# hyperledger-labs/bdls

Hardware: AMD Instinct MI355X
Metric: P-256 ECDSA verifies/sec (fused SHA-256, bit-exact vs Go crypto/ecdsa + Fabric low-S) (higher is better)
Workload: dtype u32; 1 GPU; BASELINE config 2: 1048576 records/GPU, 256B messages, 65536 distinct keys, 1/16 corrupted, fused SHA-256; records_per_gpu=1048576, records_total=1048576, msg_len=256, nkeys=65536, corrupt_den=16, parallelism=shard1 (no collective)

## Files before the change

bdls_amd/csrc/ec30.h:

```cpp
#pragma once
#include "fp30.h"

namespace bh {

struct J30 {
  uint32_t X[9], Y[9], Z[9];
};

BH_HD void j_copy(J30& r, const J30& p) {
  f_copy(r.X, p.X);
  f_copy(r.Y, p.Y);
  f_copy(r.Z, p.Z);
}

BH_HD void j_sel(J30& r, bool c, const J30& a, const J30& b) {
  f_sel(r.X, c, a.X, b.X);
  f_sel(r.Y, c, a.Y, b.Y);
  f_sel(r.Z, c, a.Z, b.Z);
}

template <class F>
BH_HD void j_dbl(J30& r, const J30& p) {
  if constexpr (F::a_is_minus3) {
    uint32_t delta[9], gamma[9], bt[9], t0[9], t1[9], u[9], alpha[9];
// ... 109 lines not shown
  f_mul<F>(t3, t2, t3);
  f_sub<F, 32>(r.Y, t3, p.Y);
  f_mul<F>(r.Z, p.Z, t1);
  f_copy(p.X, w1);
  f_copy(p.Z, r.Z);
}

template <class F>
BH_HD bool j_degenerate(const uint32_t z3[9], const uint32_t rr[9], bool* same_y) {
  const bool degenerate = f_is_zero2<F>(z3);
  if (degenerate) {
    uint32_t t[9];
    f_reduce<F>(t, rr);
    uint32_t z = 0;
    for (int i = 0; i < 9; i++) z |= t[i];
    *same_y = (z == 0);
  } else {
    *same_y = false;
  }
  return degenerate;
}

template <class F, bool FUSE = true>
BH_HD void j_zaddc(J30& r, const uint32_t x1[9], const uint32_t y1[9], const uint32_t x2[9],
                   const uint32_t dx[9], const uint32_t sy[9], const uint32_t z[9]) {
  uint32_t c[9], w1[9], w2[9], t2[9], d[9], t3[9], t4[9];
  f_sqr<F>(c, dx);
  f_mul<F>(w1, x1, c);
  f_mul<F>(w2, x2, c);
  f_dblsub<F, 32>(t2, y1, sy);
  f_sqr<F>(d, t2);
  f_sub2<F, 32>(r.X, d, w1, w2);
  f_sub<F, 64>(t3, w1, r.X);
  if constexpr (F::sparse_p256 && FUSE) {
    f_sub<F, 32>(t4, w2, w1);
    f_mul2<F>(r.Y, t2, t3, y1, t4);
  } else {
    f_sub<F, 32>(t4, w1, w2);
    f_mul<F>(t4, y1, t4);
    f_mul<F>(t3, t2, t3);
    f_sub<F, 32>(r.Y, t3, t4);
  }
  f_mul<F>(r.Z, z, dx);
}

template <class F, bool DA>
BH_HD bool j_add_impl(J30& r, const J30& p, const J30& q, bool neg, bool* same_y) {
  uint32_t z1z1[9], z2z2[9], u1[9], u2[9], s1[9], s2[9], h[9], rr[9], t[9], hh[9], hhh[9], w[9];
  f_sqr<F>(z1z1, p.Z);
  f_sqr<F>(z2z2, q.Z);
  f_mul<F>(u1, p.X, z2z2);
  f_mul<F>(u2, q.X, z1z1);
  f_mul<F>(t, q.Z, z2z2);
  f_mul<F>(s1, p.Y, t);
  f_mul<F>(t, p.Z, z1z1);
  f_mul<F>(s2, q.Y, t);
  f_sub<F, 32>(h, u2, u1);
  f_csub<F, 32>(rr, neg, s2, s1);
  f_sqr<F>(hh, h);
  f_mul<F>(hhh, hh, h);
  f_mul<F>(u1, u1, hh);
  f_sqr<F>(t, rr);
  f_add2x(w, hhh, u1);
  if constexpr (DA) {
    uint32_t x3[9], z3[9];
    f_sub<F, 32>(x3, t, w);
    f_addsub<F, 32>(u2, w, u1, t);
    f_mul<F>(s2, rr, u2);
    f_mul<F>(s1, s1, hhh);
    f_mul<F>(t, p.Z, q.Z);
    f_mul<F>(z3, t, h);
    if (j_degenerate<F>(z3, rr, same_y)) return true;
    j_zaddc<F, false>(r, u1, s1, x3, u2, s2, z3);
    return false;
  } else {
    f_sub<F, 32>(r.X, t, w);
    f_addsub<F, 32>(u2, w, u1, t);
    if constexpr (F::sparse_p256) {
      f_neg<F, 32>(s2, s1);
      f_mul2<F>(r.Y, rr, u2, s2, hhh);
    } else {
      f_mul<F>(u2, rr, u2);
      f_mul<F>(s1, s1, hhh);
      f_sub<F, 32>(r.Y, u2, s1);
    }
    f_mul<F>(t, p.Z, q.Z);
    f_mul<F>(r.Z, t, h);
    return j_degenerate<F>(r.Z, rr, same_y);
  }
}

template <class F>
BH_HD bool j_add(J30& r, const J30& p, const J30& q, bool* same_y) {
  return j_add_impl<F, false>(r, p, q, false, same_y);
}
template <class F>
BH_HD bool j_add_da(J30& r, const J30& p, const J30& q, bool* same_y, bool neg = false) {
  return j_add_impl<F, true>(r, p, q, neg, same_y);
}

template <class F, bool DA>
BH_HD bool j_madd_impl(J30& r, const J30& p, const uint32_t x2[9], const uint32_t y2[9], bool neg,
                       bool* same_y) {
  uint32_t z1z1[9], u2[9], s2[9], h[9], rr[9], t[9], hh[9], hhh[9], v[9], w[9];
  f_sqr<F>(z1z1, p.Z);
  f_mul<F>(u2, x2, z1z1);
  f_mul<F>(t, p.Z, z1z1);
  f_mul<F>(s2, y2, t);
  f_sub<F, 64>(h, u2, p.X);
  f_csub<F, 96>(rr, neg, s2, p.Y);
  f_sqr<F>(hh, h);
  f_mul<F>(hhh, hh, h);
  f_mul<F>(v, p.X, hh);
  f_sqr<F>(t, rr);
  f_add2x(w, hhh, v);
  if constexpr (DA) {
    uint32_t x3[9], z3[9];
    f_sub<F, 32>(x3, t, w);
    f_addsub<F, 32>(u2, w, v, t);
    f_mul<F>(s2, rr, u2);
    f_mul<F>(t, p.Y, hhh);
    f_mul<F>(z3, p.Z, h);
    if (j_degenerate<F>(z3, rr, same_y)) return true;
    j_zaddc<F>(r, v, t, x3, u2, s2, z3);
    return false;
  } else {
    f_sub<F, 32>(r.X, t, w);
    f_addsub<F, 32>(s2, w, v, t);
    if constexpr (F::sparse_p256) {
      f_negk<F, 96>(u2, p.Y);
      f_mul2<F>(r.Y, rr, s2, u2, hhh);
    } else {
      f_mul<F>(s2, rr, s2);
      f_mul<F>(t, p.Y, hhh);
      f_sub<F, 32>(r.Y, s2, t);
    }
    f_mul<F>(r.Z, p.Z, h);
    return j_degenerate<F>(r.Z, rr, same_y);
  }
}

template <class F>
BH_HD bool j_madd(J30& r, const J30& p, const uint32_t x2[9], const uint32_t y2[9], bool* same_y,
                  bool neg = false) {
  return j_madd_impl<F, false>(r, p, x2, y2, neg, same_y);
}
template <class F>
BH_HD bool j_madd_da(J30& r, const J30& p, const uint32_t x2[9], const uint32_t y2[9],
                     bool* same_y, bool neg = false) {
  return j_madd_impl<F, true>(r, p, x2, y2, neg, same_y);
}

template <class F>
BH_HD bool j_on_curve(const uint32_t x[9], const uint32_t y[9]) {
  uint32_t l[9], rhs[9], t[9], b[9];
  f_sqr<F>(l, y);
  f_sqr<F>(t, x);
  f_mul<F>(rhs, t, x);
  if constexpr (F::a_is_minus3) {
    f_mulc<3>(t, x);
    f_sub<F, 32>(rhs, rhs, t);
  }
  f_const(b, F::b_m);
  f_add(rhs, rhs, b);
  f_reduce<F>(rhs, rhs);
  f_canon<F>(l, l);
  return f_eq(l, rhs);
}

}
```

bdls_amd/csrc/verify.h:

```cpp
#pragma once
#include <type_traits>

#include "blake2b.h"
#include "der.h"
#include "fe.h"
#include "ec30.h"
#include "sha256.h"
#include "sha3.h"

namespace bh {

enum : uint32_t {
  BHF_HASH_SHA256 = 1u,
  BHF_NO_LOW_S = 2u,
  BHF_HASH_SHA3_256 = 8u,
  BHF_BDLS_PREHASHED = 0x100u,
};

enum : int { HK_GIVEN_OR_SHA256 = 0, HK_SHA3_256 = 1 };

enum : uint8_t { ST_R2OK = 0x80u };

struct BatchIn {
  const uint8_t* pub;
// ... 85 lines not shown
#endif
constexpr int kGW = BH_GCOMB_BITS;
static_assert(kGW >= 8 && kGW <= 14, "G comb window width");
constexpr int kCombWindows = (257 + kGW - 1) / kGW;
constexpr int kCombEntries = 1 << (kGW - 1);
static_assert(kCombWindows * kGW <= 288, "recoded scalar fits 9 limbs");
constexpr int kGEntry = 18;
constexpr int kQTab = 16;
constexpr int kQPt = 28;

struct alignas(16) W4 {
  uint32_t x, y, z, w;
};

#ifndef BH_AOS
#define BH_AOS 1
#endif
BH_HD void ld8(uint32_t v[8], const uint32_t* base, uint32_t i, uint32_t ns) {
#if BH_AOS
  const W4* p = reinterpret_cast<const W4*>(base + (size_t)i * 8);
  const W4 a = p[0], b = p[1];
  v[0] = a.x; v[1] = a.y; v[2] = a.z; v[3] = a.w;
  v[4] = b.x; v[5] = b.y; v[6] = b.z; v[7] = b.w;
#else
#pragma unroll
  for (int k = 0; k < 8; k++) v[k] = base[(size_t)k * ns + i];
#endif
}
BH_HD void st8(uint32_t* base, uint32_t i, uint32_t ns, const uint32_t v[8]) {
#if BH_AOS
  W4* p = reinterpret_cast<W4*>(base + (size_t)i * 8);
  p[0] = W4{v[0], v[1], v[2], v[3]};
  p[1] = W4{v[4], v[5], v[6], v[7]};
#else
#pragma unroll
  for (int k = 0; k < 8; k++) base[(size_t)k * ns + i] = v[k];
#endif
}
BH_HD void ld9(uint32_t v[9], const uint32_t* base, uint32_t i, uint32_t ns) {
#pragma unroll
  for (int k = 0; k < 9; k++) v[k] = BH_AOS ? base[(size_t)i * 9 + k] : base[(size_t)k * ns + i];
}
BH_HD void st9(uint32_t* base, uint32_t i, uint32_t ns, const uint32_t v[9]) {
#pragma unroll
  for (int k = 0; k < 9; k++) (BH_AOS ? base[(size_t)i * 9 + k] : base[(size_t)k * ns + i]) = v[k];
}

template <class P, class C>
BH_HD bool key_import(const uint8_t* q, uint32_t qx30[9], uint32_t qy30[9]) {
  uint32_t qx[8], qy[8], pp[8];
  load_const8(pp, C::p);
  be32_to_limbs(qx, q);
  be32_to_limbs(qy, q + 32);
  if (geq8(qx, pp) || geq8(qy, pp)) return false;
  f_from_u256(qx30, qx);
  f_from_u256(qy30, qy);
  f_to_mont<P>(qx30, qx30);
  f_to_mont<P>(qy30, qy30);
  f_canon<P>(qx30, qx30);
  f_canon<P>(qy30, qy30);
  return j_on_curve<P>(qx30, qy30);
}

template <class P, class C>
BH_HD void stage_prep_key(const BatchIn& in, const Work& w, uint32_t i) {
  uint32_t qx30[9], qy30[9];
  const bool ok = key_import<P, C>(in.pub + (size_t)i * 64, qx30, qy30);
  if (!ok) {
    f_const(qx30, P::gx_m);
    f_const(qy30, P::gy_m);
  }
  st9(w.qx, i, w.ns, qx30);
  st9(w.qy, i, w.ns, qy30);
  w.st[i] = ok ? (uint8_t)R_OK : (uint8_t)R_BAD_KEY;
}

template <class C, int HK>
BH_HD void digest_e(const BatchIn& in, uint32_t i, uint32_t e[8]) {
  const uint32_t mlen = in.msg_len[i];
  const bool fused = HK == HK_SHA3_256 || (in.flags & BHF_HASH_SHA256) != 0;
  const uint8_t* m = in.msg + in.msg_off[i];
  const uint32_t mlen2 = in.msg2_len ? in.msg2_len[i] : 0u;
  if constexpr (HK == HK_SHA3_256) {
    uint8_t hb[32];
    if (mlen2) sha3_256_msg2(hb, m, mlen, in.msg + in.msg2_off[i], mlen2);
    else sha3_256_msg(hb, m, mlen);
    be32_to_limbs(e, hb);
  } else if (fused) {
    uint32_t h[8];
    if (mlen2) sha256_msg2(h, m, mlen, in.msg + in.msg2_off[i], mlen2);
    else sha256_msg(h, m, mlen);
#pragma unroll
    for (int k = 0; k < 8; k++) e[k] = h[7 - k];
  } else {
    const uint32_t L = mlen < 32 ? mlen : 32;
#pragma unroll
    for (int k = 0; k < 8; k++) e[k] = 0;
#pragma unroll
    for (int j = 0; j < 32; j++) {
      uint32_t v = 0;
      if ((uint32_t)j < L) v = m[L - 1 - j];
      e[j >> 2] |= v << (8 * (j & 3));
    }
  }
  uint32_t nn[8], t[8];
  load_const8(nn, C::n);
  const uint32_t bo = sub8(t, e, nn);
  if (!bo) copy8(e, t);
}

template <class P, class N, class C, int HK = HK_GIVEN_OR_SHA256, bool DEFER = false>
BH_HD void stage_prep(const BatchIn& in, const Work& w, uint32_t i) {
  uint8_t reason = R_OK;
  uint32_t r[8], s[8], e[8];
  uint32_t qx30[9], qy30[9];
  const uint32_t slen = in.sig_len[i];
  const uint32_t mlen = in.msg_len[i];
  const bool fused = HK == HK_SHA3_256 || (in.flags & BHF_HASH_SHA256) != 0;
  if (slen == 0) reason = R_EMPTY_SIG;
  else if (!fused && mlen == 0) reason = R_EMPTY_DIGEST;
  DerSig ds;
  if (reason == R_OK) reason = der_parse_sig(in.sig + in.sig_off[i], slen, &ds);
  uint32_t half[8], nn[8];
  load_const8(half, C::half_n);
  load_const8(nn, C::n);
  if (reason == R_OK) {
    copy8(r, ds.r);
    copy8(s, ds.s);
    if (!(in.flags & BHF_NO_LOW_S) && (ds.s_big || !geq8(half, s))) reason = R_HIGH_S;
  }
  if (reason == R_OK && !key_import<P, C>(in.pub + (size_t)i * 64, qx30, qy30))
    reason = R_BAD_KEY;
  if (reason == R_OK && (ds.r_big || geq8(r, nn))) reason = R_R_RANGE;
  if (reason == R_OK && (ds.s_big || geq8(s, nn))) reason = R_S_RANGE;
  if (reason == R_OK && !DEFER) digest_e<C, HK>(in, i, e);
  uint8_t st = reason;
  if (reason == R_OK) {
    uint32_t pmn[8], rn[8], rm[9], r2m[9];
    load_const8(pmn, C::p_minus_n);
    f_from_u256(rm, r);
    f_to_mont<P>(rm, rm);
    f_canon<P>(rm, rm);
    if (!geq8(r, pmn)) {
      st |= ST_R2OK;
      add8(rn, r, nn);
      f_from_u256(r2m, rn);
      f_to_mont<P>(r2m, r2m);
      f_canon<P>(r2m, r2m);
    } else {
      f_copy(r2m, rm);
    }
    st9(w.rm, i, w.ns, rm);
    st9(w.r2m, i, w.ns, r2m);
    to_mont<N>(s, s);
  } else {
    for (int k = 0; k < 8; k++) { e[k] = r[k] = 0; }
    e[0] = r[0] = 1;
    load_const8(s, N::r1);
    f_const(qx30, P::gx_m);
    f_const(qy30, P::gy_m);
  }
  if (!DEFER) st8(w.e, i, w.ns, e);
  st8(w.r, i, w.ns, r);
  st8(w.sm, i, w.ns, s);
  st9(w.qx, i, w.ns, qx30);
  st9(w.qy, i, w.ns, qy30);
  w.st[i] = st;
}

BH_HD void setbytes_u256(const uint8_t* b, uint32_t len, uint32_t v[8], bool* big, bool* zero) {
  uint32_t lo = 0;
  while (lo < len && b[lo] == 0) lo++;
  const uint32_t L = len - lo;
  *zero = (L == 0);
  *big = (L > 32);
#pragma unroll
  for (int k = 0; k < 8; k++) v[k] = 0;
  if (L > 32) return;
#pragma unroll
  for (int j = 0; j < 32; j++) {
    uint32_t x = 0;
    if ((uint32_t)j < L) x = b[len - 1 - j];
    v[j >> 2] |= x << (8 * (j & 3));
  }
}

template <class C>
BH_HD void stage_bdls_given(const BdlsIn& in, const Work& w, uint32_t i) {
  uint32_t e[8], nn[8], t[8];
  const uint8_t* m = in.msg + in.msg_off[i];
  const uint32_t mlen = in.msg_len[i];
  const uint32_t L = mlen < 32 ? mlen : 32;
#pragma unroll
  for (int k = 0; k < 8; k++) e[k] = 0;
#pragma unroll
  for (int j = 0; j < 32; j++) {
    uint32_t v = 0;
    if ((uint32_t)j < L) v = m[L - 1 - j];
    e[j >> 2] |= v << (8 * (j & 3));
  }
  load_const8(nn, C::n);
  if (!sub8(t, e, nn)) copy8(e, t);
  st8(w.e, i, w.ns, e);
}

template <class C>
BH_HD void stage_bdls_hash(const BdlsIn& in, const Work& w, uint32_t i) {
  if (in.flags & BHF_BDLS_PREHASHED) return stage_bdls_given<C>(in, w, i);
  uint8_t hsh[32];
  uint32_t e[8], nn[8], t[8];
  const uint8_t* q = in.xy + (size_t)i * 64;
  bdls_signed_proto_hash(hsh, in.version[i], q, q + 32, in.msg + in.msg_off[i], in.msg_len[i]);
  be32_to_limbs(e, hsh);
  load_const8(nn, C::n);
  if (!sub8(t, e, nn)) copy8(e, t);
  st8(w.e, i, w.ns, e);
}

template <class P, class N, class C>
BH_HD void stage_prep(const BdlsIn& in, const Work& w, uint32_t i) {
  uint8_t reason = R_OK;
  uint32_t r[8], s[8], nn[8];
  uint32_t qx30[9], qy30[9];
  load_const8(nn, C::n);
  bool rbig, rzero, sbig, szero;
  setbytes_u256(in.r + in.r_off[i], in.r_len[i], r, &rbig, &rzero);
  setbytes_u256(in.s + in.s_off[i], in.s_len[i], s, &sbig, &szero);
  if (rzero) reason = R_R_NONPOS;
  else if (szero) reason = R_S_NONPOS;
  const uint8_t* q = in.xy + (size_t)i * 64;
  const bool badkey = reason == R_OK && !key_import<P, C>(q, qx30, qy30);
  if (badkey && P::a_is_minus3) reason = R_BAD_KEY;
  if (reason == R_OK && (rbig || geq8(r, nn))) reason = R_R_RANGE;
  if (reason == R_OK && (sbig || geq8(s, nn))) reason = R_S_RANGE;
  if (reason == R_OK && badkey) reason = R_MATH;
  uint8_t st = reason;
  if (reason == R_OK) {
    uint32_t pmn[8], rn[8], rm[9], r2m[9];
    load_const8(pmn, C::p_minus_n);
    f_from_u256(rm, r);
    f_to_mont<P>(rm, rm);
    f_canon<P>(rm, rm);
    if (!geq8(r, pmn)) {
      st |= ST_R2OK;
      add8(rn, r, nn);
      f_from_u256(r2m, rn);
      f_to_mont<P>(r2m, r2m);
      f_canon<P>(r2m, r2m);
    } else {
      f_copy(r2m, rm);
    }
    st9(w.rm, i, w.ns, rm);
    st9(w.r2m, i, w.ns, r2m);
    to_mont<N>(s, s);
  } else {
    for (int k = 0; k < 8; k++) r[k] = 0;
    r[0] = 1;
    load_const8(s, N::r1);
    f_const(qx30, P::gx_m);
    f_const(qy30, P::gy_m);
  }
  st8(w.r, i, w.ns, r);
  st8(w.sm, i, w.ns, s);
  st9(w.qx, i, w.ns, qx30);
  st9(w.qy, i, w.ns, qy30);
  w.st[i] = st;
}

template <class N, bool U1 = true, bool VAR = false>
BH_HD void stage_inv(const Work& w, uint32_t c, uint32_t stride, uint32_t n) {
  uint32_t acc[8], x[8];
  load_const8(acc, N::r1);
  uint32_t last = c;
  for (uint32_t i = c; i < n; i += stride) {
    st8(w.pre, i, w.ns, acc);
    ld8(x, w.sm, i, w.ns);
    mont_mul<N>(acc, acc, x);
    last = i;
  }
  if (c >= n) return;
  uint32_t inv[8];
  mont_inv_sg<N, VAR>(inv, acc);
  for (uint32_t i = last;; i -= stride) {
    uint32_t pre[8], wi[8], t[8];
    ld8(pre, w.pre, i, w.ns);
    mont_mul<N>(wi, inv, pre);
    ld8(x, w.sm, i, w.ns);
    mont_mul<N>(inv, inv, x);
    if constexpr (U1) {
      ld8(t, w.e, i, w.ns);
      mont_mul<N>(t, t, wi);
      st8(w.e, i, w.ns, t);
    } else {
      st8(w.sm, i, w.ns, wi);
    }
    ld8(t, w.r, i, w.ns);
    mont_mul<N>(t, t, wi);
    st8(w.r, i, w.ns, t);
    if (i < c + stride) break;
  }
}

template <class N>
BH_HD void calc_u1(uint32_t u1[8], const Work& w, uint32_t i) {
  uint32_t wi[8];
  ld8(u1, w.e, i, w.ns);
  ld8(wi, w.sm, i, w.ns);
  mont_mul<N>(u1, u1, wi);
}

BH_HD void booth5(uint32_t in6, uint32_t* mag, bool* neg) {
  uint32_t sgn = 0u - (in6 >> 5);
  uint32_t d = (63u - in6) & sgn;
  d |= in6 & ~sgn;
  *mag = (d >> 1) + (d & 1u);
  *neg = sgn != 0;
}


BH_HD uint32_t* qtab_entry(uint32_t* tab, uint32_t wave, uint32_t entry, uint32_t lane) {
  return tab + (((size_t)wave * 64 + lane) * kQTab + entry) * kQPt;
}

BH_HD void qtab_store(uint32_t* tab, uint32_t wave, uint32_t entry, uint32_t lane, const J30& P) {
  uint32_t v[28];
#pragma unroll
  for (int k = 0; k < 9; k++) {
    v[k] = P.X[k];
    v[9 + k] = P.Y[k];
    v[18 + k] = P.Z[k];
  }
  v[27] = 0;
  W4* d = reinterpret_cast<W4*>(qtab_entry(tab, wave, entry, lane));
#pragma unroll
  for (int q = 0; q < 7; q++) d[q] = W4{v[4 * q], v[4 * q + 1], v[4 * q + 2], v[4 * q + 3]};
}

BH_HD void qtab_load(J30& P, const uint32_t* tab, uint32_t wave, uint32_t entry, uint32_t lane) {
  const W4* s = reinterpret_cast<const W4*>(qtab_entry(const_cast<uint32_t*>(tab), wave, entry, lane));
  uint32_t v[28];
#pragma unroll
  for (int q = 0; q < 7; q++) {
    const W4 t = s[q];
    v[4 * q] = t.x;
    v[4 * q + 1] = t.y;
    v[4 * q + 2] = t.z;
    v[4 * q + 3] = t.w;
  }
#pragma unroll
  for (int k = 0; k < 9; k++) {
    P.X[k] = v[k];
    P.Y[k] = v[9 + k];
    P.Z[k] = v[18 + k];
  }
}

template <class P>
BH_HD void gtab_entry(uint32_t t, uint32_t* out) {
  const uint32_t win = t / kCombEntries, j = t % kCombEntries;
  J30 B;
  f_const(B.X, P::gx_m);
  f_const(B.Y, P::gy_m);
  f_const(B.Z, P::r1);
  for (uint32_t d = 0; d < (uint32_t)kGW * win; d++) j_dbl<P>(B, B);
  const uint32_t k = j + 1;
  int top = 31;
  while (!((k >> top) & 1u)) top--;
  J30 A;
  j_copy(A, B);
  for (int b = top - 1; b >= 0; b--) {
    j_dbl<P>(A, A);
    if ((k >> b) & 1u) {
      bool same;
      J30 R;
      j_add<P>(R, A, B, &same);
      j_copy(A, R);
    }
  }
  uint32_t zi[9], zi2[9], x[9], y[9], z[9];
  f_reduce<P>(z, A.Z);
  f_inv<P>(zi, z);
  f_sqr<P>(zi2, zi);
  f_mul<P>(x, A.X, zi2);
  f_mul<P>(zi2, zi2, zi);
  f_mul<P>(y, A.Y, zi2);
  f_reduce<P>(x, x);
  f_reduce<P>(y, y);
  for (int q = 0; q < 9; q++) {
    out[q] = x[q];
    out[9 + q] = y[q];
  }
}

template <int B>
BH_HD void shr_const(uint32_t v[9]) {
  constexpr int ws = B / 32, bs = B % 32;
#pragma unroll
  for (int q = 0; q < 9; q++) {
    const uint32_t lo = (q + ws < 9) ? v[q + ws] : 0u;
    const uint32_t hi = (q + ws + 1 < 9) ? v[q + ws + 1] : 0u;
    if constexpr (bs != 0) v[q] = (lo >> bs) | (hi << (32 - bs));
    else v[q] = lo;
  }
}

struct GOff {
  uint32_t v[9];
};
constexpr GOff make_goff() {
  GOff o{};
  for (int w = 0; w < kCombWindows; w++) {
    const int b = w * kGW + kGW - 1;
    o.v[b / 32] |= 1u << (b % 32);
  }
  return o;
}
constexpr GOff kGOff = make_goff();

BH_HD void recode_goff(uint32_t v[9], const uint32_t k[8]) {
  uint64_t c = 0;
#pragma unroll
  for (int q = 0; q < 8; q++) {
    c += (uint64_t)k[q] + kGOff.v[q];
    v[q] = (uint32_t)c;
    c >>= 32;
  }
  v[8] = (uint32_t)c + kGOff.v[8];
}

#ifndef BH_GCOMB_PREFETCH
#define BH_GCOMB_PREFETCH 1
#endif
BH_HD void g_window(uint32_t v[9], int win, const uint32_t* gtab, uint32_t tx[9], uint32_t ty[9],
                    uint32_t& mag, bool& neg) {
  const int d = (int)(v[0] & (2u * kCombEntries - 1u)) - kCombEntries;
// ... 875 lines not shown
constexpr size_t kG2Words = (size_t)(kG2Ent + kG1Ent + kGBase) * kLLAff;
constexpr size_t kGCombWords = (size_t)kCombWindows * kCombEntries * kGEntry;
constexpr size_t kGTabAllWords = kGCombWords + kG2Words;
static_assert(kGCombWords % 4 == 0, "folded tables 16-byte aligned");
BH_HD const uint32_t* g2_of(const uint32_t* gtab) { return gtab + kGCombWords; }

template <class P>
BH_HD void scalar_g_affine(const uint32_t v[9], uint32_t x[9], uint32_t y[9]) {
  uint32_t gx[9], gy[9];
  f_const(gx, P::gx_m);
  f_const(gy, P::gy_m);
  int topbit = 287;
  while (topbit > 0 && !((v[topbit >> 5] >> (topbit & 31)) & 1u)) topbit--;
  J30 A;
  f_copy(A.X, gx);
  f_copy(A.Y, gy);
  f_const(A.Z, P::r1);
  for (int b = topbit - 1; b >= 0; b--) {
    j_dbl<P>(A, A);
    if ((v[b >> 5] >> (b & 31)) & 1u) {
      bool same;
      (void)j_madd<P>(A, A, gx, gy, &same);
    }
  }
  uint32_t z[9], zi[9], zi2[9];
  f_reduce<P>(z, A.Z);
  f_inv<P>(zi, z);
  f_sqr<P>(zi2, zi);
  f_mul<P>(x, A.X, zi2);
  f_mul<P>(zi2, zi2, zi);
  f_mul<P>(y, A.Y, zi2);
  f_reduce<P>(x, x);
  f_reduce<P>(y, y);
}

template <class P>
BH_HD void gtab2_base(uint32_t k, uint32_t* g2) {
  const uint32_t i = k / kGOdd, m = k % kGOdd;
  uint32_t v[9] = {0, 0, 0, 0, 0, 0, 0, 0, 0};
  const int b = kLLSpace * (int)i;
  const uint64_t mag = (uint64_t)(2u * m + 1u) << (b & 31);
  v[b >> 5] = (uint32_t)mag;
  if ((b >> 5) + 1 < 9) v[(b >> 5) + 1] = (uint32_t)(mag >> 32);
  uint32_t x[9], y[9];
  scalar_g_affine<P>(v, x, y);
  llaff_store(g2, kG2Ent + kG1Ent + k, x, y);
}

template <class P>
BH_HD void gtab2_entry(uint32_t t, uint32_t* g2) {
  constexpr uint32_t top = 1u << (kLLTeeth - 1), all = (1u << kLLTeeth) - 1u;
  int c[kLLTeeth];
  for (int i = 0; i < kLLTeeth; i++) c[i] = 0;
  if (t < kG2Ent) {
    for (int cc = 0; cc < kGF; cc++) {
      const uint32_t bits = cc == kGF - 1 ? (top | (t >> ((kGF - 1) * kLLTeeth)))
                                          : (t >> (cc * kLLTeeth)) & all;
      for (int i = 0; i < kLLTeeth; i++) c[i] += (2 * (int)((bits >> i) & 1u) - 1) << cc;
    }
  } else {
    const uint32_t b = top | (t - kG2Ent);
    for (int i = 0; i < kLLTeeth; i++) c[i] = 2 * (int)((b >> i) & 1u) - 1;
  }
  J30 A;
  llaff_load(A.X, A.Y, g2, kG2Ent + kG1Ent + (uint32_t)(kLLTeeth - 1) * kGOdd +
                               (uint32_t)((c[kLLTeeth - 1] - 1) / 2));
  f_const(A.Z, P::r1);
  for (int i = kLLTeeth - 2; i >= 0; i--) {
    const int a = c[i] < 0 ? -c[i] : c[i];
    uint32_t bx[9], by[9];
    llaff_load(bx, by, g2, kG2Ent + kG1Ent + (uint32_t)i * kGOdd + (uint32_t)((a - 1) / 2));
    if (c[i] < 0) f_neg<P, 64>(by, by);
    bool same;
    (void)j_madd<P>(A, A, bx, by, &same);
  }
  uint32_t zi[9], x[9], y[9];
  f_inv_sg<P>(zi, A.Z);
  ll_to_affine<P>(x, y, A, zi);
  llaff_store(g2, t, x, y);
}

BH_HD void g2_column(const uint64_t gl[kLLTeeth], int j, uint32_t& idx, bool& neg) {
  if (j == 0) {
    ll_column(gl, 0, idx, neg);
    idx += kG2Ent;
    return;
  }
  constexpr uint32_t all = (1u << kLLTeeth) - 1u;
  uint32_t col[kGF];
#pragma unroll
  for (int cc = 0; cc < kGF; cc++) {
    uint32_t b = 0;
#pragma unroll
    for (int t = 0; t < kLLTeeth; t++) b |= (uint32_t)((gl[t] >> (j + cc)) & 1ull) << t;
    col[cc] = b;
  }
  neg = ((col[kGF - 1] >> (kLLTeeth - 1)) & 1u) == 0u;
  uint32_t x = col[kGF - 1] & (all >> 1);
  if (neg) x = ~col[kGF - 1] & (all >> 1);
#pragma unroll
  for (int cc = kGF - 2; cc >= 0; cc--) x = (x << kLLTeeth) | ((neg ? ~col[cc] : col[cc]) & all);
  idx = x;
}

template <class P>
BH_HD void ll_madd(J30& A, bool& a_inf, const uint32_t tx[9], uint32_t ty[9], bool neg,
                   const uint32_t one[9]) {
  bool same;
  const bool deg = j_madd<P>(A, A, tx, ty, &same, neg);
  if (a_inf || deg) {
    if (neg) f_neg<P, 64>(ty, ty);
    if (a_inf || same) {
      J30 T;
      f_copy(T.X, tx);
      f_copy(T.Y, ty);
      f_copy(T.Z, one);
      if (a_inf) j_copy(A, T);
      else j_dbl<P>(A, T);
      a_inf = false;
    } else {
      a_inf = true;
    }
  }
}

template <class P>
BH_HD void ll_dbladd(J30& A, bool& a_inf, const uint32_t tx[9], uint32_t ty[9], bool neg,
                     const uint32_t one[9]) {
  if (a_inf) {
    if (neg) f_neg<P, 64>(ty, ty);
    f_copy(A.X, tx);
    f_copy(A.Y, ty);
    f_copy(A.Z, one);
    a_inf = false;
    return;
  }
  bool same;
  if (j_madd_da<P>(A, A, tx, ty, &same, neg)) {
    if (neg) f_neg<P, 64>(ty, ty);
    J30 T;
    f_copy(T.X, tx);
    f_copy(T.Y, ty);
    f_copy(T.Z, one);
    if (same) {
      j_dbl<P>(A, T);
      (void)j_madd<P>(A, A, tx, ty, &same);
    }
    return;
  }
  if (f_is_zero2<P>(A.Z)) a_inf = true;
}

template <class P>
BH_HD void q_llcomb_g(J30& A, bool& a_inf, const Work& w, uint32_t i, const uint32_t* tab,
                      uint32_t stride, const uint32_t* g2) {
  uint32_t u2[8], u1[8], one[9];
  ld8(u2, w.r, i, w.ns);
  ld8(u1, w.e, i, w.ns);
  f_const(one, P::r1);
  uint64_t sl[kLLTeeth], gl[kLLTeeth];
  ll_slices<P>(sl, u2);
  ll_slices<P>(gl, u1);
  uint32_t idx;
  bool neg;
  ll_column(sl, kLLSpace - 1, idx, neg);
  if (stride) llent_load(A.X, A.Y, tab + idx * stride);
  else llaff_load(A.X, A.Y, tab, idx);
  f_copy(A.Z, one);
  a_inf = false;
  uint32_t gx[9], gy[9], gidx;
  bool gneg;
  g2_column(gl, kLLSpace - kGF, gidx, gneg);
  llaff_load(gx, gy, g2, gidx);
#pragma unroll 1
  for (int j = kLLSpace - 2; j >= 0; j--) {
    {
      uint32_t tx[9], ty[9];
      ll_column(sl, j, idx, neg);
      if (stride) llent_load(tx, ty, tab + idx * stride);
      else llaff_load(tx, ty, tab, idx);
      ll_dbladd<P>(A, a_inf, tx, ty, neg, one);
    }
    if (j == 0 || (j - 1) % kGF == 0) {
      ll_madd<P>(A, a_inf, gx, gy, gneg, one);
      if (j > 0) {
        g2_column(gl, j > kGF ? j - kGF : 0, gidx, gneg);
        llaff_load(gx, gy, g2, gidx);
      }
    }
  }
}

template <class P>
BH_HD bool stage_keycomb_fold(const Work& w, uint32_t i, const uint32_t* tab, uint32_t stride,
                              const uint32_t* g2) {
  J30 A;
  bool a_inf;
  q_llcomb_g<P>(A, a_inf, w, i, tab, stride, g2);
  return finish_check<P>(w, i, A, a_inf, A, true);
}

#ifndef BH_LADDER_CSUB
#define BH_LADDER_CSUB 1
#endif
template <class P>
BH_HD void j_dbladd(J30& A, bool& a_inf, J30& T, bool neg) {
  if (a_inf) {
    if (neg) f_neg<P, 64>(T.Y, T.Y);
    j_copy(A, T);
    a_inf = false;
    return;
  }
  bool same;
  if (j_add_da<P>(A, A, T, &same, neg)) {
    if (neg) f_neg<P, 64>(T.Y, T.Y);
    if (same) {
      J30 D;
      j_dbl<P>(D, T);
      (void)j_add<P>(A, D, T, &same);
    }
    return;
  }
  if (f_is_zero2<P>(A.Z)) a_inf = true;
}

BH_HD bool g_fold_pos(int p) { return p == 0 || (p >= 1 && p <= kLLSpace - kGF && (p - 1) % kGF == 0); }

template <class P>
BH_HD void q_ladder_odd_g(J30& A, bool& a_inf, const Work& w, uint32_t i, uint32_t wave,
                          uint32_t lane, const uint32_t* g2) {
  using Cv = CvOf<P>;
  uint32_t u2[8], u1[8], qx[9], qy[9], one[9];
  ld8(u2, w.r, i, w.ns);
  ld8(u1, w.e, i, w.ns);
  ld9(qx, w.qx, i, w.ns);
  ld9(qy, w.qy, i, w.ns);
  f_const(one, P::r1);
  {
    J30 Qa, D, S;
    f_copy(Qa.X, qx);
    f_copy(Qa.Y, qy);
    f_copy(Qa.Z, one);
    j_dblu<P>(D, S, Qa);
    qtab_store(w.qtab, wave, 0, lane, S);
#pragma unroll 1
    for (uint32_t m = 1; m < (uint32_t)kQTab; m++) {
      J30 Sn;
      j_zaddu<P>(Sn, D, S);
      qtab_store(w.qtab, wave, m, lane, Sn);
      j_copy(S, Sn);
    }
  }
  uint32_t K[9];
  {
    const uint32_t add = (u2[0] & 1u) ? 0u : ~0u;
    uint32_t k[9];
    uint64_t cy = 0;
#pragma unroll
    for (int q = 0; q < 8; q++) {
      cy += (uint64_t)u2[q] + (Cv::n[q] & add);
      k[q] = (uint32_t)cy;
      cy >>= 32;
    }
    k[8] = (uint32_t)cy;
    K[0] = k[0] << 30;
#pragma unroll
    for (int q = 1; q < 9; q++) K[q] = (k[q] << 30) | (k[q - 1] >> 2);
  }
  uint64_t gl[kLLTeeth];
  ll_slices<P>(gl, u1);
  uint32_t gx[9], gy[9], gidx;
  bool gneg;
  int gp = kLLSpace - kGF;
  g2_column(gl, gp, gidx, gneg);
  llaff_load(gx, gy, g2, gidx);
  auto g_add = [&]() {
    ll_madd<P>(A, a_inf, gx, gy, gneg, one);
    if (gp > 0) {
      gp = gp > kGF ? gp - kGF : 0;
      g2_column(gl, gp, gidx, gneg);
      llaff_load(gx, gy, g2, gidx);
    }
  };
  qtab_load(A, w.qtab, wave, (K[8] >> 30) & 1u, lane);
  a_inf = false;
#pragma unroll 1
  for (int win = 50; win >= 0; win--) {
    const uint32_t b = (K[8] >> 25) & 31u;
#pragma unroll
    for (int q = 8; q > 0; q--) K[q] = (K[q] << 5) | (K[q - 1] >> 27);
    K[0] <<= 5;
    const bool neg = b < 16u;
    const uint32_t mag = neg ? 31u - 2u * b : 2u * b - 31u;
    J30 T;
    qtab_load(T, w.qtab, wave, (mag - 1u) >> 1, lane);
#pragma unroll 1
    for (int d = 1; d <= 4; d++) {
      j_dbl<P>(A, A);
      if (g_fold_pos(5 * win + 5 - d)) g_add();
    }
#if BH_LADDER_CSUB
    j_dbladd<P>(A, a_inf, T, neg);
#else
    if (neg) f_neg<P, 64>(T.Y, T.Y);
    j_dbladd<P>(A, a_inf, T, false);
#endif
    if (g_fold_pos(5 * win)) g_add();
  }
}

template <class P>
BH_HD bool stage_ladder_fold(const Work& w, const uint32_t* gtab, uint32_t i, uint32_t wave,
                             uint32_t lane) {
  if constexpr (P::a_is_minus3) {
    J30 A;
    bool a_inf;
    q_ladder_odd_g<P>(A, a_inf, w, i, wave, lane, g2_of(gtab));
    return finish_check<P>(w, i, A, a_inf, A, true);
  } else {
    return stage_ladder<P>(w, gtab, i, wave, lane);
  }
}

template <class P>
BH_HD bool stage_keycomb(const Work& w, const uint32_t* gtab, uint32_t i, const uint32_t* tab,
                         bool aff = false) {
  J30 A, B;
  bool a_inf, b_inf;
  q_keycomb<P>(A, a_inf, w, i, tab, aff);
  uint32_t u1[8];
  ld8(u1, w.e, i, w.ns);
  g_comb<P>(B, b_inf, gtab, u1);
  return finish_check<P>(w, i, A, a_inf, B, b_inf);
}

constexpr uint32_t kGPartWords = 28;
template <class P>
BH_HD void stage_gpart(const Work& w, const uint32_t* gtab, uint32_t i, uint32_t j) {
  J30 B;
  bool b_inf;
  uint32_t u1[8];
  ld8(u1, w.e, i, w.ns);
// ... 280 lines not shown
```

bdls_amd/csrc/fe.h:

```cpp
#pragma once
#include "bh_common.h"
#include "curve_consts.h"

namespace bh {

BH_HD uint32_t add8(uint32_t r[8], const uint32_t a[8], const uint32_t b[8]) {
  uint32_t c = 0;
#pragma unroll
  for (int i = 0; i < 8; i++) r[i] = __builtin_addc(a[i], b[i], c, &c);
  return c;
}

BH_HD uint32_t sub8(uint32_t r[8], const uint32_t a[8], const uint32_t b[8]) {
  uint32_t c = 0;
#pragma unroll
  for (int i = 0; i < 8; i++) r[i] = __builtin_subc(a[i], b[i], c, &c);
  return c;
}

BH_HD bool geq8(const uint32_t a[8], const uint32_t b[8]) {
  uint32_t c = 0;
#pragma unroll
  for (int i = 0; i < 8; i++) (void)__builtin_subc(a[i], b[i], c, &c);
  return c == 0;
}

BH_HD bool is_zero8(const uint32_t a[8]) {
  uint32_t x = 0;
#pragma unroll
  for (int i = 0; i < 8; i++) x |= a[i];
  return x == 0;
}

BH_HD bool eq8(const uint32_t a[8], const uint32_t b[8]) {
  uint32_t x = 0;
#pragma unroll
  for (int i = 0; i < 8; i++) x |= a[i] ^ b[i];
  return x == 0;
}

BH_HD void copy8(uint32_t r[8], const uint32_t a[8]) {
#pragma unroll
  for (int i = 0; i < 8; i++) r[i] = a[i];
}

BH_HD void sel8(uint32_t r[8], bool c, const uint32_t a[8], const uint32_t b[8]) {
#pragma unroll
  for (int i = 0; i < 8; i++) r[i] = c ? a[i] : b[i];
}

template <class C>
BH_HD void load_const8(uint32_t r[8], const C& c) {
#pragma unroll
  for (int i = 0; i < 8; i++) r[i] = c[i];
}

template <class M>
BH_HD void mod_add(uint32_t r[8], const uint32_t a[8], const uint32_t b[8]) {
  uint32_t s[8], d[8];
  uint32_t c = add8(s, a, b);
  uint32_t bo = 0;
#pragma unroll
  for (int i = 0; i < 8; i++) d[i] = __builtin_subc(s[i], M::m[i], bo, &bo);
  bool use_d = c | (bo ^ 1u);
  sel8(r, use_d, d, s);
}

template <class M>
BH_HD void mod_sub(uint32_t r[8], const uint32_t a[8], const uint32_t b[8]) {
  uint32_t d[8], e[8];
  uint32_t bo = sub8(d, a, b);
  uint32_t c = 0;
#pragma unroll
  for (int i = 0; i < 8; i++) e[i] = __builtin_addc(d[i], M::m[i], c, &c);
  sel8(r, bo != 0, e, d);
}

template <class M>
BH_HD void mod_dbl(uint32_t r[8], const uint32_t a[8]) { mod_add<M>(r, a, a); }

template <class M>
BH_HD void mod_neg(uint32_t r[8], const uint32_t a[8]) {
  uint32_t z[8] = {0, 0, 0, 0, 0, 0, 0, 0};
  mod_sub<M>(r, z, a);
}

template <class M>
BH_HD void mont_mul(uint32_t r[8], const uint32_t a[8], const uint32_t b[8]) {
  uint32_t t[8] = {0, 0, 0, 0, 0, 0, 0, 0};
  uint32_t t8 = 0;
#pragma unroll
  for (int i = 0; i < 8; i++) {
    uint64_t c = 0;
#pragma unroll
    for (int j = 0; j < 8; j++) {
      uint64_t uv = (uint64_t)a[j] * b[i] + t[j] + c;
      t[j] = (uint32_t)uv;
      c = uv >> 32;
    }
    uint64_t uv = (uint64_t)t8 + c;
    t8 = (uint32_t)uv;
    uint32_t t9 = (uint32_t)(uv >> 32);
    const uint32_t m = t[0] * M::n0;
    uv = (uint64_t)m * M::m[0] + t[0];
    c = uv >> 32;
#pragma unroll
    for (int j = 1; j < 8; j++) {
      uv = (uint64_t)m * M::m[j] + t[j] + c;
      t[j - 1] = (uint32_t)uv;
      c = uv >> 32;
    }
    uv = (uint64_t)t8 + c;
    t[7] = (uint32_t)uv;
    t8 = t9 + (uint32_t)(uv >> 32);
  }
  uint32_t d[8];
  uint32_t bo = 0;
#pragma unroll
  for (int i = 0; i < 8; i++) d[i] = __builtin_subc(t[i], M::m[i], bo, &bo);
  bool use_d = (t8 != 0) | (bo == 0);
  sel8(r, use_d, d, t);
}

template <class M>
BH_HD void mont_sqr(uint32_t r[8], const uint32_t a[8]) {
  mont_mul<M>(r, a, a);
}

template <class M>
BH_HD void to_mont(uint32_t r[8], const uint32_t a[8]) {
  uint32_t r2[8];
  load_const8(r2, M::r2);
  mont_mul<M>(r, a, r2);
}

template <class M>
BH_HD void from_mont(uint32_t r[8], const uint32_t a[8]) {
  uint32_t one[8] = {1, 0, 0, 0, 0, 0, 0, 0};
  mont_mul<M>(r, a, one);
}

template <class M>
BH_HDNI void mont_inv(uint32_t r[8], const uint32_t a[8]) {
  uint32_t acc[8];
  load_const8(acc, M::r1);
  for (int i = 255; i >= 0; i--) {
    mont_sqr<M>(acc, acc);
    if ((M::mm2[i >> 5] >> (i & 31)) & 1u) mont_mul<M>(acc, acc, a);
  }
  copy8(r, acc);
}

struct Div2x2 {
  int32_t u, v, q, r;
};

BH_HD int32_t divsteps30(int32_t zeta, uint32_t f, uint32_t g, Div2x2& t) {
  uint32_t u = 1, v = 0, q = 0, r = 1;
#pragma unroll
  for (int i = 0; i < 30; i++) {
    uint32_t m1 = (uint32_t)(zeta >> 31);
    const uint32_t m2 = 0u - (g & 1u);
    const uint32_t x = (f ^ m1) - m1, y = (u ^ m1) - m1, z = (v ^ m1) - m1;
    g += x & m2;
    q += y & m2;
    r += z & m2;
    m1 &= m2;
    zeta = (zeta ^ (int32_t)m1) - 1;
    f += g & m1;
    u += q & m1;
    v += r & m1;
    g >>= 1;
    u <<= 1;
    v <<= 1;
  }
  t.u = (int32_t)u;
  t.v = (int32_t)v;
  t.q = (int32_t)q;
  t.r = (int32_t)r;
  return zeta;
}

BH_HD int32_t divsteps30_var(int32_t eta, uint32_t f, uint32_t g, Div2x2& t) {
  uint32_t u = 1, v = 0, q = 0, r = 1;
  int i = 30;
  for (;;) {
    const int zeros = __builtin_ctz(g | (0xffffffffu << i));
    g >>= zeros;
    u <<= zeros;
    v <<= zeros;
    eta -= zeros;
    i -= zeros;
    if (i == 0) break;
    if (eta < 0) {
      const uint32_t x = f, y = u, z = v;
      eta = -eta;
      f = g;
      u = q;
      v = r;
      g = 0u - x;
      q = 0u - y;
      r = 0u - z;
    }
    int limit = eta + 1 < i ? eta + 1 : i;
    if (limit > 6) limit = 6;
    const uint32_t m = (0xffffffffu >> (32 - limit)) & 63u;
    const uint32_t finv = f * (2u - f * f);
    const uint32_t w = (0u - g * finv) & m;
    g += f * w;
    q += u * w;
    r += v * w;
  }
  t.u = (int32_t)u;
  t.v = (int32_t)v;
  t.q = (int32_t)q;
  t.r = (int32_t)r;
  return eta;
}

constexpr int32_t kS30Mask = 0x3fffffff;

template <class M>
BH_HD void divsteps_update_de(int32_t d[9], int32_t e[9], const Div2x2& t) {
  const int32_t sd = d[8] >> 31, se = e[8] >> 31;
  int32_t md = (t.u & sd) + (t.v & se);
  int32_t me = (t.q & sd) + (t.r & se);
  int64_t cd = (int64_t)t.u * d[0] + (int64_t)t.v * e[0];
  int64_t ce = (int64_t)t.q * d[0] + (int64_t)t.r * e[0];
  md -= (int32_t)((M::inv30 * (uint32_t)cd + (uint32_t)md) & (uint32_t)kS30Mask);
  me -= (int32_t)((M::inv30 * (uint32_t)ce + (uint32_t)me) & (uint32_t)kS30Mask);
  cd += (int64_t)M::s30[0] * md;
  ce += (int64_t)M::s30[0] * me;
  cd >>= 30;
  ce >>= 30;
#pragma unroll
  for (int i = 1; i < 9; i++) {
    const int32_t di = d[i], ei = e[i];
    cd += (int64_t)t.u * di + (int64_t)t.v * ei + (int64_t)M::s30[i] * md;
    ce += (int64_t)t.q * di + (int64_t)t.r * ei + (int64_t)M::s30[i] * me;
    d[i - 1] = (int32_t)cd & kS30Mask;
    e[i - 1] = (int32_t)ce & kS30Mask;
    cd >>= 30;
    ce >>= 30;
  }
  d[8] = (int32_t)cd;
  e[8] = (int32_t)ce;
}

BH_HD void divsteps_update_fg(int32_t f[9], int32_t g[9], const Div2x2& t) {
  int64_t cf = (int64_t)t.u * f[0] + (int64_t)t.v * g[0];
  int64_t cg = (int64_t)t.q * f[0] + (int64_t)t.r * g[0];
  cf >>= 30;
  cg >>= 30;
#pragma unroll
  for (int i = 1; i < 9; i++) {
    const int32_t fi = f[i], gi = g[i];
    cf += (int64_t)t.u * fi + (int64_t)t.v * gi;
    cg += (int64_t)t.q * fi + (int64_t)t.r * gi;
    f[i - 1] = (int32_t)cf & kS30Mask;
    g[i - 1] = (int32_t)cg & kS30Mask;
    cf >>= 30;
    cg >>= 30;
  }
  f[8] = (int32_t)cf;
  g[8] = (int32_t)cg;
}

template <class M>
BH_HD void s30_addm_neg(int32_t d[9], bool c, bool neg) {
  int64_t cy = 0;
#pragma unroll
  for (int i = 0; i < 9; i++) {
    int64_t v = (int64_t)d[i] + (c ? M::s30[i] : 0);
    cy += neg ? -v : v;
    if (i < 8) {
      d[i] = (int32_t)cy & kS30Mask;
      cy >>= 30;
    } else {
      d[8] = (int32_t)cy;
    }
  }
}

template <class M, bool VAR = false>
BH_HD void mod_inv_sg(uint32_t r[8], const uint32_t a[8]) {
  int32_t d[9] = {0, 0, 0, 0, 0, 0, 0, 0, 0};
  int32_t e[9] = {1, 0, 0, 0, 0, 0, 0, 0, 0};
  int32_t f[9], g[9];
#pragma unroll
  for (int i = 0; i < 9; i++) {
    f[i] = M::s30[i];
    const int b = 30 * i, w = b >> 5, s = b & 31;
    uint64_t x = a[w];
    if (w + 1 < 8) x |= (uint64_t)a[w + 1] << 32;
    g[i] = (int32_t)((x >> s) & (i < 8 ? (uint64_t)kS30Mask : 0xffffffffull));
  }
  int32_t zeta = -1;
  for (int it = 0; it < (VAR ? 25 : 20); it++) {
    Div2x2 t;
    if constexpr (VAR) {
      int32_t any = 0;
#pragma unroll
      for (int k = 0; k < 9; k++) any |= g[k];
      if (!any) break;
      zeta = divsteps30_var(zeta, (uint32_t)f[0], (uint32_t)g[0], t);
    } else {
      zeta = divsteps30(zeta, (uint32_t)f[0], (uint32_t)g[0], t);
    }
    divsteps_update_de<M>(d, e, t);
    divsteps_update_fg(f, g, t);
  }
  s30_addm_neg<M>(d, d[8] < 0, f[8] < 0);
  s30_addm_neg<M>(d, d[8] < 0, false);
#pragma unroll
  for (int w = 0; w < 8; w++) {
    const int b = 32 * w, i = b / 30, s = b % 30;
    uint64_t x = (uint64_t)(uint32_t)d[i] >> s;
    if (i + 1 < 9) x |= (uint64_t)(uint32_t)d[i + 1] << (30 - s);
    r[w] = (uint32_t)x;
  }
}

template <class M, bool VAR = false>
BH_HD void mont_inv_sg(uint32_t r[8], const uint32_t a[8]) {
  uint32_t t[8], r3[8];
  mod_inv_sg<M, VAR>(t, a);
  load_const8(r3, M::r3);
  mont_mul<M>(r, t, r3);
}

BH_HD void be32_to_limbs(uint32_t r[8], const uint8_t* b) {
#pragma unroll
  for (int i = 0; i < 8; i++) {
    const uint8_t* p = b + 28 - 4 * i;
    r[i] = ((uint32_t)p[0] << 24) | ((uint32_t)p[1] << 16) | ((uint32_t)p[2] << 8) | p[3];
  }
}

BH_HD void limbs_to_be32(uint8_t* b, const uint32_t a[8]) {
#pragma unroll
  for (int i = 0; i < 8; i++) {
    uint8_t* p = b + 28 - 4 * i;
    p[0] = (uint8_t)(a[i] >> 24);
    p[1] = (uint8_t)(a[i] >> 16);
    p[2] = (uint8_t)(a[i] >> 8);
    p[3] = (uint8_t)a[i];
  }
}

}
```

Baseline: 208.7 million verifies/s.

## Fuse G-table addition with key-table point via affine pre-add in comb loop

At comb columns where a generator-table point is also added, the two affine points (key table and G table) are first summed into a Z-bearing point, and then a single double-and-add with that combined point is applied to the accumulator. This replaces a separate dbl-add plus mixed add with one pre-add and one Jacobian double-add that reuses the precomputed Z^2/Z^3 from the pre-add. The loop is restructured into an inner run of plain dbladd steps and a G-step. It falls back to the old path when the accumulator is infinity or the addition degenerates, which adds branch divergence and extra code size or register pressure.

```diff
diff --git a/bdls_amd/csrc/ec30.h b/bdls_amd/csrc/ec30.h
--- a/bdls_amd/csrc/ec30.h
+++ b/bdls_amd/csrc/ec30.h
@@ -285,6 +285,59 @@
 }
 
 template <class F>
+BH_HD bool a_preadd(J30& u, uint32_t hh[9], uint32_t hhh[9], const uint32_t tx[9],
+                    const uint32_t ty[9], const uint32_t gx[9], const uint32_t gy[9], bool neg) {
+  uint32_t rr[9], v[9], t[9], w[9], d[9];
+  f_sub<F, 64>(u.Z, gx, tx);
+  f_csub<F, 96>(rr, neg, gy, ty);
+  f_sqr<F>(hh, u.Z);
+  f_mul<F>(hhh, hh, u.Z);
+  f_mul<F>(v, tx, hh);
+  f_sqr<F>(t, rr);
+  f_add2x(w, hhh, v);
+  f_sub<F, 32>(u.X, t, w);
+  f_addsub<F, 32>(d, w, v, t);
+  if constexpr (F::sparse_p256) {
+    f_negk<F, 96>(w, ty);
+    f_mul2<F>(u.Y, rr, d, w, hhh);
+  } else {
+    f_mul<F>(d, rr, d);
+    f_mul<F>(t, ty, hhh);
+    f_sub<F, 32>(u.Y, d, t);
+  }
+  return f_is_zero2<F>(hh);
+}
+
+template <class F, bool FUSE>
+BH_HD bool j_add_da_z(J30& r, const J30& p, const J30& q, const uint32_t z2z2[9],
+                      const uint32_t z2z3[9], bool neg, bool* same_y) {
+  uint32_t z1z1[9], u1[9], u2[9], s1[9], s2[9], h[9], rr[9], t[9], hh[9], hhh[9], w[9];
+  uint32_t x3[9], z3[9];
+  f_sqr<F>(z1z1, p.Z);
+  f_mul<F>(u1, p.X, z2z2);
+  f_mul<F>(u2, q.X, z1z1);
+  f_mul<F>(s1, p.Y, z2z3);
+  f_mul<F>(t, p.Z, z1z1);
+  f_mul<F>(s2, q.Y, t);
+  f_sub<F, 32>(h, u2, u1);
+  f_csub<F, 32>(rr, neg, s2, s1);
+  f_sqr<F>(hh, h);
+  f_mul<F>(hhh, hh, h);
+  f_mul<F>(u1, u1, hh);
+  f_sqr<F>(t, rr);
+  f_add2x(w, hhh, u1);
+  f_sub<F, 32>(x3, t, w);
+  f_addsub<F, 32>(u2, w, u1, t);
+  f_mul<F>(s2, rr, u2);
+  f_mul<F>(s1, s1, hhh);
+  f_mul<F>(t, p.Z, q.Z);
+  f_mul<F>(z3, t, h);
+  if (j_degenerate<F>(z3, rr, same_y)) return true;
+  j_zaddc<F, FUSE>(r, u1, s1, x3, u2, s2, z3);
+  return false;
+}
+
+template <class F>
 BH_HD bool j_on_curve(const uint32_t x[9], const uint32_t y[9]) {
   uint32_t l[9], rhs[9], t[9], b[9];
   f_sqr<F>(l, y);
diff --git a/bdls_amd/csrc/verify.h b/bdls_amd/csrc/verify.h
--- a/bdls_amd/csrc/verify.h
+++ b/bdls_amd/csrc/verify.h
@@ -1571,6 +1571,30 @@
 }
 
 template <class P>
+BH_HD bool ll_gfuse(J30& A, bool& a_inf, const uint32_t tx[9], const uint32_t ty[9], bool neg,
+                    const uint32_t gx[9], const uint32_t gy[9], bool gneg) {
+  J30 U;
+  uint32_t hh[9], hhh[9];
+  bool same;
+  (void)a_preadd<P>(U, hh, hhh, tx, ty, gx, gy, neg != gneg);
+  if (j_add_da_z<P, true>(A, A, U, hh, hhh, neg, &same)) return false;
+  if (f_is_zero2<P>(A.Z)) a_inf = true;
+  return true;
+}
+
+template <class P>
+BH_HD void ll_step_g(J30& A, bool& a_inf, const uint32_t tx[9], uint32_t ty[9], bool neg,
+                     const uint32_t gx[9], uint32_t gy[9], bool gneg, bool gstep,
+                     const uint32_t one[9]) {
+  bool done = false;
+  if (gstep && !a_inf) done = ll_gfuse<P>(A, a_inf, tx, ty, neg, gx, gy, gneg);
+  if (!done) {
+    ll_dbladd<P>(A, a_inf, tx, ty, neg, one);
+    if (gstep) ll_madd<P>(A, a_inf, gx, gy, gneg, one);
+  }
+}
+
+template <class P>
 BH_HD void q_llcomb_g(J30& A, bool& a_inf, const Work& w, uint32_t i, const uint32_t* tab,
                       uint32_t stride, const uint32_t* g2) {
   uint32_t u2[8], u1[8], one[9];
@@ -1591,22 +1615,29 @@
   bool gneg;
   g2_column(gl, kLLSpace - kGF, gidx, gneg);
   llaff_load(gx, gy, g2, gidx);
+  int j = kLLSpace - 2;
 #pragma unroll 1
-  for (int j = kLLSpace - 2; j >= 0; j--) {
+  while (j >= 0) {
+#pragma unroll 1
+    for (; j > 0 && (j - 1) % kGF != 0; j--) {
+      uint32_t tx[9], ty[9];
+      ll_column(sl, j, idx, neg);
+      if (stride) llent_load(tx, ty, tab + idx * stride);
+      else llaff_load(tx, ty, tab, idx);
+      ll_dbladd<P>(A, a_inf, tx, ty, neg, one);
+    }
     {
       uint32_t tx[9], ty[9];
       ll_column(sl, j, idx, neg);
       if (stride) llent_load(tx, ty, tab + idx * stride);
       else llaff_load(tx, ty, tab, idx);
-      ll_dbladd<P>(A, a_inf, tx, ty, neg, one);
-    }
-    if (j == 0 || (j - 1) % kGF == 0) {
-      ll_madd<P>(A, a_inf, gx, gy, gneg, one);
-      if (j > 0) {
-        g2_column(gl, j > kGF ? j - kGF : 0, gidx, gneg);
-        llaff_load(gx, gy, g2, gidx);
-      }
-    }
+      ll_step_g<P>(A, a_inf, tx, ty, neg, gx, gy, gneg, true, one);
+    }
+    if (j > 0) {
+      g2_column(gl, j > kGF ? j - kGF : 0, gidx, gneg);
+      llaff_load(gx, gy, g2, gidx);
+    }
+    j--;
   }
 }
 
```

Measured after the change: 210.5 million verifies/s (median of 6 runs). No clear change (+0.8%).

## Reimplement Montgomery multiplication with 30-bit limbs and column-wise lazy reduction

Applied to the files above, without the earlier changes.

Montgomery multiplication now converts its 8x32-bit operands to 9x30-bit limbs and pre-shifts them so that R=2^270 behaves as 2^256. It then does a product-scanning schoolbook multiply into 64-bit column accumulators with deferred carries, interleaves the reduction, and converts back to 8x32 with one final conditional subtract. A compile-time check confirms that no column can overflow 64 bits, and the reduction constants are forced into scalar registers. Separately, the batch inversion now works on non-Montgomery s values with a plain modular inverse plus one multiply by R^2, which removes the per-record to_mont conversion. The goal is fewer carry-chain dependencies per multiply, at the cost of more multiplies (81 vs 64) and extra slicing and repacking work.

```diff
diff --git a/bdls_amd/csrc/fe.h b/bdls_amd/csrc/fe.h
--- a/bdls_amd/csrc/fe.h
+++ b/bdls_amd/csrc/fe.h
@@ -85,41 +85,117 @@
   mod_sub<M>(r, z, a);
 }
 
+constexpr int32_t kS30Mask = 0x3fffffff;
+constexpr int kMmShA = 7, kMmShB = 7;
+static_assert(kMmShA + kMmShB == 270 - 256, "the pre-shifts turn R = 2^270 into 2^256");
+
+template <class M>
+constexpr bool mm_cols_fit() {
+  typedef unsigned __int128 u128;
+  const u128 full = (1u << 30) - 1;
+  u128 A[9] = {}, B[9] = {};
+  for (int i = 0; i < 8; i++) A[i] = B[i] = full;
+  A[8] = (1u << (16 + kMmShA)) - 1;
+  B[8] = (1u << (16 + kMmShB)) - 1;
+  u128 carry = 0;
+  for (int k = 0; k < 17; k++) {
+    u128 col = carry;
+    for (int i = 0; i < 9; i++)
+      if (k - i >= 0 && k - i < 9) col += A[i] * B[k - i];
+    for (int j = 0; j < 9; j++)
+      if (k - j >= 0 && k - j < 9) col += full * (u128)(uint32_t)M::s30[k - j];
+    if (col >> 64) return false;
+    carry = col >> 30;
+  }
+  return true;
+}
+
+template <int SH>
+BH_HD void mm_slice(uint32_t r[9], const uint32_t a[8]) {
+  r[0] = (a[0] << SH) & (uint32_t)kS30Mask;
+#pragma unroll
+  for (int i = 1; i < 9; i++) {
+    const int lo = 30 * i - SH;
+    const int w = lo >> 5, s = lo & 31;
+    uint32_t v = a[w] >> s;
+    if (s > 2 && w + 1 < 8) v |= a[w + 1] << (32 - s);
+    r[i] = i < 8 ? v & (uint32_t)kS30Mask : v;
+  }
+}
+
+template <uint32_t K>
+BH_HD void mm_mac(uint64_t& c, uint32_t x) {
+#if defined(__HIP_DEVICE_COMPILE__)
+  uint32_t k = K;
+  asm("" : "+s"(k));
+  c += (uint64_t)x * k;
+#else
+  c += (uint64_t)x * K;
+#endif
+}
+
+template <class M, int J>
+BH_HD void mm_redc_row(uint64_t* C, uint32_t mk) {
+  if constexpr (J < 9) {
+    if constexpr (M::s30[J] != 0) mm_mac<(uint32_t)M::s30[J]>(C[J], mk);
+    mm_redc_row<M, J + 1>(C, mk);
+  }
+}
+
+template <class M>
+BH_HD void mm_mul9(uint32_t t[9], const uint32_t a[9], const uint32_t b[9]) {
+  static_assert(mm_cols_fit<M>(), "mont_mul: a column of the product can pass 2^64");
+  static_assert(M::s30[8] < (1 << 16), "mont_mul: m < 2^256");
+  constexpr uint32_t n0 = (0u - M::inv30) & (uint32_t)kS30Mask;
+  uint64_t C[17];
+#pragma unroll
+  for (int k = 0; k < 17; k++) C[k] = 0;
+#pragma unroll
+  for (int i = 0; i < 9; i++)
+#pragma unroll
+    for (int j = 0; j < 9; j++) C[i + j] += (uint64_t)a[i] * b[j];
+  uint64_t acc = 0;
+#pragma unroll
+  for (int k = 0; k < 17; k++) {
+    acc += C[k];
+    if (k < 9) {
+      const uint32_t mk = ((uint32_t)acc * n0) & (uint32_t)kS30Mask;
+      mm_mac<(uint32_t)M::s30[0]>(acc, mk);
+      mm_redc_row<M, 1>(C + k, mk);
+    } else {
+      t[k - 9] = (uint32_t)acc & (uint32_t)kS30Mask;
+    }
+    acc >>= 30;
+  }
+  t[8] = (uint32_t)acc;
+}
+
+template <class M>
+BH_HD void mm_canon8(uint32_t r[8], const uint32_t t[9]) {
+  uint32_t v[8], d[8];
+#pragma unroll
+  for (int w = 0; w < 8; w++) {
+    const int bit = 32 * w;
+    const int i = bit / 30, s = bit % 30;
+    uint32_t x = t[i] >> s;
+    if (i + 1 < 9) x |= t[i + 1] << (30 - s);
+    v[w] = x;
+  }
+  const uint32_t top = t[8] >> 16;
+  uint32_t bo = 0;
+#pragma unroll
+  for (int i = 0; i < 8; i++) d[i] = __builtin_subc(v[i], M::m[i], bo, &bo);
+  const bool use_d = (top != 0) | (bo == 0);
+  sel8(r, use_d, d, v);
+}
+
 template <class M>
 BH_HD void mont_mul(uint32_t r[8], const uint32_t a[8], const uint32_t b[8]) {
-  uint32_t t[8] = {0, 0, 0, 0, 0, 0, 0, 0};
-  uint32_t t8 = 0;
-#pragma unroll
-  for (int i = 0; i < 8; i++) {
-    uint64_t c = 0;
-#pragma unroll
-    for (int j = 0; j < 8; j++) {
-      uint64_t uv = (uint64_t)a[j] * b[i] + t[j] + c;
-      t[j] = (uint32_t)uv;
-      c = uv >> 32;
-    }
-    uint64_t uv = (uint64_t)t8 + c;
-    t8 = (uint32_t)uv;
-    uint32_t t9 = (uint32_t)(uv >> 32);
-    const uint32_t m = t[0] * M::n0;
-    uv = (uint64_t)m * M::m[0] + t[0];
-    c = uv >> 32;
-#pragma unroll
-    for (int j = 1; j < 8; j++) {
-      uv = (uint64_t)m * M::m[j] + t[j] + c;
-      t[j - 1] = (uint32_t)uv;
-      c = uv >> 32;
-    }
-    uv = (uint64_t)t8 + c;
-    t[7] = (uint32_t)uv;
-    t8 = t9 + (uint32_t)(uv >> 32);
-  }
-  uint32_t d[8];
-  uint32_t bo = 0;
-#pragma unroll
-  for (int i = 0; i < 8; i++) d[i] = __builtin_subc(t[i], M::m[i], bo, &bo);
-  bool use_d = (t8 != 0) | (bo == 0);
-  sel8(r, use_d, d, t);
+  uint32_t a9[9], b9[9], t[9];
+  mm_slice<kMmShA>(a9, a);
+  mm_slice<kMmShB>(b9, b);
+  mm_mul9<M>(t, a9, b9);
+  mm_canon8<M>(r, t);
 }
 
 template <class M>
@@ -218,8 +294,6 @@
   return eta;
 }
 
-constexpr int32_t kS30Mask = 0x3fffffff;
-
 template <class M>
 BH_HD void divsteps_update_de(int32_t d[9], int32_t e[9], const Div2x2& t) {
   const int32_t sd = d[8] >> 31, se = e[8] >> 31;
diff --git a/bdls_amd/csrc/verify.h b/bdls_amd/csrc/verify.h
--- a/bdls_amd/csrc/verify.h
+++ b/bdls_amd/csrc/verify.h
@@ -261,11 +261,9 @@
     }
     st9(w.rm, i, w.ns, rm);
     st9(w.r2m, i, w.ns, r2m);
-    to_mont<N>(s, s);
   } else {
-    for (int k = 0; k < 8; k++) { e[k] = r[k] = 0; }
-    e[0] = r[0] = 1;
-    load_const8(s, N::r1);
+    for (int k = 0; k < 8; k++) { e[k] = r[k] = s[k] = 0; }
+    e[0] = r[0] = s[0] = 1;
     f_const(qx30, P::gx_m);
     f_const(qy30, P::gy_m);
   }
@@ -361,11 +359,9 @@
     }
     st9(w.rm, i, w.ns, rm);
     st9(w.r2m, i, w.ns, r2m);
-    to_mont<N>(s, s);
   } else {
-    for (int k = 0; k < 8; k++) r[k] = 0;
-    r[0] = 1;
-    load_const8(s, N::r1);
+    for (int k = 0; k < 8; k++) r[k] = s[k] = 0;
+    r[0] = s[0] = 1;
     f_const(qx30, P::gx_m);
     f_const(qy30, P::gy_m);
   }
@@ -378,8 +374,7 @@
 
 template <class N, bool U1 = true, bool VAR = false>
 BH_HD void stage_inv(const Work& w, uint32_t c, uint32_t stride, uint32_t n) {
-  uint32_t acc[8], x[8];
-  load_const8(acc, N::r1);
+  uint32_t acc[8] = {1, 0, 0, 0, 0, 0, 0, 0}, x[8];
   uint32_t last = c;
   for (uint32_t i = c; i < n; i += stride) {
     st8(w.pre, i, w.ns, acc);
@@ -388,8 +383,10 @@
     last = i;
   }
   if (c >= n) return;
-  uint32_t inv[8];
-  mont_inv_sg<N, VAR>(inv, acc);
+  uint32_t inv[8], r2[8];
+  mod_inv_sg<N, VAR>(inv, acc);
+  load_const8(r2, N::r2);
+  mont_mul<N>(inv, inv, r2);
   for (uint32_t i = last;; i -= stride) {
     uint32_t pre[8], wi[8], t[8];
     ld8(pre, w.pre, i, w.ns);
```

Measured after the change: 207.8 million verifies/s before, 208.7 million verifies/s after (median of 4 runs). Within noise of the previous version (+0.5%).
